# sczhou/CodeFormer

Hardware: AMD Instinct MI355X
Metric: aligned 512x512 faces/sec (whole node) at w=0.5 (higher is better)
Workload: dtype f32; 1 GPU; BASELINE config 2 (IEEE fp32 arithmetic): 16 faces/GPU, w=0.5, adain, seed-0 random-init weights; global_batch=16, parallelism=single GPU, precision=fp32

## Files before the change

### codeformer_amd/archs/codeformer_arch.py

```python
import gc
import os
import threading

import math
import numbers

import numpy as np
import torch
import torch.nn.functional as F
from torch import nn

from .. import ops
from ..ops import EPI_GELU, EPI_RESIDUAL, EPI_SFT, PRO_LEAKY
from ..utils.diagnostics import top2_gap
from ..utils.registry import ARCH_REGISTRY
from .hip_module import PACK_EPOCH, HipModule
from .vqgan_arch import ResBlock, VQAutoEncoder


_GRAPH_LOCK = threading.RLock()
_CAPTURE_STREAMS = {}


def _min_nan(a, b):
# ... 286 lines not shown
    def _encode_hip(self, x, code_only, adain, f43_encoder=None, guard=False, u8=False):
        if u8:
            B = x.shape[0]
        else:
            B, _, Himg, Wimg = x.shape
            if (Himg, Wimg) != (512, 512):
                raise ValueError(f'CodeFormer expects aligned 512x512 faces, got {Himg}x{Wimg}')
            x = x.float().contiguous()
        enc_feat = {}
        enc_taps = {self.fuse_encoder_block[f]: (lambda t: enc_feat.__setitem__(str(t.shape[2]), t))
                    for f in self.connect_list}
        if self.encoder_precision not in ('auto', 'fp32', 'f16x2'):
            raise ValueError(f"encoder_precision must be 'auto', 'fp32' or 'f16x2', got {self.encoder_precision!r}")
        enc_code = ops.SPLIT if self.encoder_precision == 'f16x2' or (self.encoder_precision == 'auto' and self.precision != 'fp32') else ops.WINOGRAD
        if self.winograd_f43_encoder if f43_encoder is None else f43_encoder:
            enc_code = {ops.SPLIT: ops.SPLIT_F43, ops.WINOGRAD: ops.WINOGRAD_F43}[enc_code]
        lq = self.encoder.forward_nhwc(x, enc_taps, bf16=enc_code, img_u8=u8)
        T = lq.shape[1] * lq.shape[2]
        tokens = lq.view(B * T, lq.shape[3])

        if self.gemm_precision not in ('auto', 'fp32', 'f16x2'):
            raise ValueError(f"gemm_precision must be 'auto', 'fp32' or 'f16x2', got {self.gemm_precision!r}")
        gcode = ops.GSPLIT if self.gemm_precision == 'f16x2' else 0
        gcode_ln = ops.GSPLIT if (self.gemm_precision == 'f16x2' or (self.gemm_precision == 'auto' and self.precision != 'fp32' and self.encoder_precision != 'fp32')) else 0
        X = ops.linear(tokens, self._pw_conv('feat_emb', bf16=gcode))
        for layer in self.ft_layers:
            X = layer.forward_tokens(X, self.position_emb, B, code=gcode, code_ln=gcode_ln)
        ln, head = self.idx_pred_layer[0], self.idx_pred_layer[1]
        logits2d = ops.linear(ops.layernorm(X, ln.weight, ln.bias, ln.eps), self._pw_conv(head, bf16=ln_code(self, ln, gcode_ln)))
        res = {'logits': logits2d.view(B, T, -1), 'lq_feat': ops.to_nchw(lq), 'idx': None, 'quant': None, 'enc_feat': enc_feat}
        if guard:
# ... 2 lines not shown
        if code_only:
            return res

        if not guard:
            idx = ops.argmax_rows(logits2d)
            res['idx'] = idx.view(B, T)
        quant = ops.codebook_gather(idx, self.quantize.embedding.weight, B, T,
                                    lq=tokens.view(B, T, -1) if adain else None)
        res['quant'] = quant.view(B, lq.shape[1], lq.shape[2], -1)
        if self.precision not in ('fp32', 'f16x2', 'bf16', 'fp16'):
            raise ValueError(f"precision must be 'fp32', 'f16x2', 'bf16' or 'fp16', got {self.precision!r}")
        return res

    def _generate_hip(self, quant, enc_feat, w, u8=False, out_u8=None):
        B = quant.shape[0]
        bf16 = {'fp32': ops.WINOGRAD_F43, 'f16x2': ops.SPLIT_F43, 'bf16': 1, 'fp16': 2}[self.precision]
        gen_taps = None
        if (torch.is_tensor(w) and w.dim() == 1) or w > 0:
            def fuse(t):
                f = str(t.shape[2])
                enc = enc_feat[f]
                if t.dtype == torch.bfloat16:
                    enc = ops.to_bf16(enc)
                return self.fuse_convs_dict[f].forward_nhwc(enc, t, w, bf16=bf16)
            gen_taps = {self.fuse_generator_block[f]: fuse for f in self.connect_list}
        if u8 and out_u8 is None:
            out_u8 = torch.empty((B, 512, 512, 3), dtype=torch.uint8, device=quant.device)
        return self.generator.forward_nhwc(quant, gen_taps, bf16=bf16, storage_bf16=bool(self.bf16_storage) and bf16 == 1,
                                           img_out=out_u8 if u8 else None)

    def _generate_rows_hip(self, e, w, u8=False, out_u8=None):
# ... 85 lines not shown
            key = (tuple(x.shape), ('per-face', w.fused) if per_face else float(w), bool(code_only), bool(adain), self.precision, bool(self.bf16_storage), self.encoder_precision, self.gemm_precision, bool(self.winograd_f43_encoder), str(x.device), ops.switches(), bool(guard), bool(u8))
            ent = self._graphs.get(key)
            sig = self._param_signature()
            if ent is None or ent['epoch'] != PACK_EPOCH[0] or ent['sig'] != sig:
                static_x = x.clone() if u8 else x.float().contiguous().clone()
                for _ in range(2):
                    self._forward_hip(static_x, w, code_only, adain, guard=guard, u8=u8)
                torch.cuda.synchronize(x.device)
                graph = torch.cuda.CUDAGraph()
                cap = _CAPTURE_STREAMS.get(str(x.device))
                if cap is None:
                    cap = _CAPTURE_STREAMS[str(x.device)] = torch.cuda.Stream(device=x.device)
                with torch.cuda.stream(cap):
                    ops._act_cells(x.device, 4 * max(int(x.shape[0]), 1))
                    ops._counters(x.device, 4096)
                cap.synchronize()
                gc_on = gc.isenabled()
                gc.disable()
                try:
                    with torch.cuda.graph(graph, stream=cap):
                        outs = self._forward_hip(static_x, w, code_only, adain, guard=guard, u8=u8)
                finally:
                    if gc_on:
                        gc.enable()
                ent = {'graph': graph, 'x': static_x, 'outs': outs, 'epoch': PACK_EPOCH[0], 'sig': sig, 'idx': getattr(self, 'last_indices', None),
                       'gap': self.last_min_gap if guard else None, 'w': w if per_face else None}
                self.graph_captures += 1
                self._graphs.pop(key, None)
                while len(self._graphs) >= 4:
                    self._graphs.pop(next(iter(self._graphs)))
# ... 232 lines not shown
```

### codeformer_amd/archs/hip_module.py

```python
import torch
from torch import nn

from .. import ops


PACK_EPOCH = [0]


class HipModule(nn.Module):

    def _packed(self, key, build, *params):
        sig = tuple((p.data_ptr(), ops.tensor_version(p), str(p.device)) for p in params if p is not None)
        cache = self.__dict__.setdefault('_hip_cache', {})
        ent = cache.get(key)
        if ent is None or ent[0] != sig:
            ent = (sig, build())
            cache[key] = ent
            PACK_EPOCH[0] += 1
        return ent[1]

    def _pw_conv(self, name, bf16=False, up2x=False, f16=False, hw=None, c_split=None):
        conv = getattr(self, name) if isinstance(name, str) else name
        code = 2 if f16 else int(bf16)
        if code in (ops.WINOGRAD, ops.WINOGRAD_F43) + ops.SPLIT_CODES or (code in (1, 2) and hw is not None and not up2x):
            cout, cin = conv.weight.shape[:2]
            if hw is None or tuple(conv.weight.shape[2:]) != (3, 3):
                code = 0
            else:
                code = ops.conv_code(code, cin, cout, hw[0], hw[1], up2x=up2x, c_split=c_split)
        key = (name if isinstance(name, str) else id(conv), code, bool(up2x))
        return self._packed(key, lambda: ops.pack_weight(conv.weight, conv.bias, bf16=code, up2x=up2x), conv.weight, conv.bias)

    def _range_code(self, norm, code, n):
        code = int(code)
        if code in (0, 1, ops.WINOGRAD, ops.WINOGRAD_F43):
            return code
        gmax, bmax = self._packed(('gn_range', id(norm)),
                                  lambda: (float(norm.weight.detach().abs().max()), float(norm.bias.detach().abs().max())),
                                  norm.weight, norm.bias)
        return code if ops.gn_range_ok(gmax, bmax, n) else ops.exact_code(code)

    def invalidate_packed_weights(self):
        for m in self.modules():
            if isinstance(m, HipModule):
                m.__dict__.pop('_hip_cache', None)
        PACK_EPOCH[0] += 1

    def forward_nhwc(self, x):
        raise NotImplementedError

# ... 10 lines not shown
```

### codeformer_amd/archs/vqgan_arch.py

```python
import torch
import torch.nn.functional as F
from torch import nn

from .. import ops
from ..ops import EPI_RESIDUAL, PRO_AFFINE, PRO_AFFINE_SWISH
from ..utils.logger import get_root_logger
from ..utils.registry import ARCH_REGISTRY
from .hip_module import HipModule

GN_GROUPS = 32
GN_EPS = 1e-6


def normalize(in_channels):
    return nn.GroupNorm(num_groups=GN_GROUPS, num_channels=in_channels, eps=GN_EPS, affine=True)


def swish(x):
    return x * torch.sigmoid(x)


def _gn_tables(norm, *xs, act_growth=None):
    return ops.groupnorm_tables(list(xs), norm.weight, norm.bias, norm.eps, norm.num_groups, act_growth=act_growth)

# ... 72 lines not shown

    def forward_host(self, x):
        return self.conv(F.pad(x, (0, 1, 0, 1), mode='constant', value=0))


class Upsample(HipModule):

    def __init__(self, in_channels):
        super().__init__()
        self.conv = nn.Conv2d(in_channels, in_channels, kernel_size=3, stride=1, padding=1)

    def forward_nhwc(self, x, bf16=False):
        if int(bf16) == 2:
            bf16 = ops.SPLIT
        c = self.conv.in_channels
        if int(bf16) == ops.WINOGRAD_F43 and x.dtype == torch.float32 and ops.f43_up_ok(c, self.conv.out_channels, 2 * x.shape[1], 2 * x.shape[2]):
            pw = self._packed(('conv', 'f42up'), lambda: ops.pack_weight(self.conv.weight, self.conv.bias, bf16=ops.WF42U), self.conv.weight, self.conv.bias)
            return ops.conv2d(x, pw, upsample=True, emit_stats=True)
        pw = self._pw_conv('conv', bf16, up2x=True, hw=x.shape[1:3])
        return ops.conv2d(x, pw, upsample=True, emit_stats=True, act=ops.act_scale(x) if ops.needs_act_scale(pw) else None)

    def forward_host(self, x):
        return self.conv(F.interpolate(x, scale_factor=2.0, mode='nearest'))


class ResBlock(HipModule):

    def __init__(self, in_channels, out_channels=None):
        super().__init__()
        self.in_channels = in_channels
        self.out_channels = in_channels if out_channels is None else out_channels
# ... 282 lines not shown
```

### codeformer_amd/build.py

```python
import os
import shutil
import subprocess
import sys

PKG = os.path.dirname(os.path.abspath(__file__))
CSRC = os.path.join(PKG, 'csrc')
ROOT = os.path.dirname(PKG)
LIB = os.path.join(PKG, 'libcodeformer_hip.so')
SOURCES = ['cf_igemm.hip', 'cf_winograd.hip', 'cf_split.hip', 'cf_wsplit.hip', 'cf_wf43.hip', 'cf_gemm_split.hip', 'cf_pack.hip', 'cf_norm.hip', 'cf_attention.hip', 'cf_misc.hip', 'cf_paste.hip', 'cf_dcn.hip', 'cf_warp.hip', 'cf_metrics.hip', 'cf_arcface.hip', 'cf_vgg.hip', 'cf_bisenet.hip']


def _hipcc():
    for c in (os.environ.get('HIPCC'), shutil.which('hipcc'), '/opt/rocm/bin/hipcc'):
        if c and os.path.exists(c):
            return c
    raise RuntimeError('hipcc not found (set HIPCC)')


def source_hash():
    import hashlib
    h = hashlib.sha256()
    files = sorted(os.path.join(CSRC, f) for f in os.listdir(CSRC) if f.endswith(('.hip', '.h'))) + \
        [os.path.join(ROOT, 'include', 'codeformer_hip.h')]
    for f in files:
# ... 98 lines not shown
```

### codeformer_amd/csrc/cf_conv_parts.h

```cpp
#pragma once
#include <type_traits>

#include "cf_common.h"

int cf_winograd_launch(const cf_conv_desc* d, hipStream_t stream, int* parts_query, const float* sft_w_img = nullptr);
bool cf_wsplit_covers(const cf_conv_desc* d);
int cf_wsplit_launch(const cf_conv_desc* d, hipStream_t stream, int* parts_query, const float* sft_w_img = nullptr);
int cf_wf43_launch(const cf_conv_desc* d, hipStream_t stream, int* parts_query, const float* sft_w_img = nullptr);
bool cf_wf43_k32(int cout, int cin);
int cf_split_launch(const cf_conv_desc* d, hipStream_t stream, int* parts_query, const float* sft_w_img = nullptr);
int cf_gemm_split_launch(const cf_conv_desc* d, hipStream_t stream, int* parts_query);
int cf_gemm_f32_tile_try(const cf_conv_desc* d, hipStream_t stream);
int cf_gemm_split_geometry(const cf_conv_desc* d, int* tiles, long* bytes_per_part);
int cf_winograd_splitk_geometry(const cf_conv_desc* d, int* tiles, long* bytes_per_part);
int cf_split_splitk_geometry(const cf_conv_desc* d, int* tiles, long* bytes_per_part);

template <class A>
inline void cf_fill_conv_args(A& a, const cf_conv_desc* d, const float* sft_w_img = nullptr) {
  a.in0 = d->in0;
  a.in1 = d->in1;
  a.c0 = d->c0;
  a.c1 = d->c1;
  a.cin = d->c0 + d->c1;
  a.batch = d->batch;
// ... 167 lines not shown
```

### codeformer_amd/csrc/cf_wf43.hip

```cpp
#include <cstdlib>
#include <cstring>
#include <type_traits>

#include "cf_conv_parts.h"




namespace {

constexpr int F4_TH = 16, F4_TW = 16;
constexpr int F4_PW = F4_TW + 2;
constexpr int F4_NPIX = (F4_TH + 2) * F4_PW;
constexpr int F4_SLOTS = F4_NPIX + 4;
constexpr int F4_DUMMY = F4_NPIX;
constexpr int F4_NT = 16;
constexpr int F4_PATCH_FLOATS = F4_SLOTS * CF_BK;
constexpr int F4_PS = F4_NT * CF_BK;
constexpr int F4_V_FLOATS = 36 * F4_PS;
constexpr int F4_M_FLOATS = 36 * 8 * 64;
constexpr int F4_TAB = 256;
constexpr int F4_TAB_32 = 512;
constexpr int F4_LDS_FLOATS = 2 * F4_PATCH_FLOATS + F4_V_FLOATS + 2 * F4_TAB;
static_assert(F4_M_FLOATS <= 2 * F4_PATCH_FLOATS + F4_V_FLOATS, "epilogue staging must fit the patch buffers + V");
// ... 42 lines not shown
  double* stats_out;
  int stats_cpg, nparts;
  int tiles_x, tiles_per_img, ntn;
  int nt_out;
};
static_assert(sizeof(F4Args) == 168, "the kernarg block is 168 bytes (160 before sft_w_img, which found no padding to take): its size feeds the register allocation of every instantiation, so a change is re-checked with tools/kernel_resources.py");

__device__ __forceinline__ int f4_vs(int ty) { return (0x78 >> (2 * ty)) & 3; }

__device__ __forceinline__ unsigned f4_vu(unsigned lq, unsigned p, unsigned t) { return (lq & 1u) + 2u * (((t >> 1) + 4u * (lq >> 1) + p) & 7u); }

template <int PRO, int EPI, int NW, int KS, bool F32, int UPF = 0>
__global__ __launch_bounds__(NW * 64, 4) void wf43_kernel(const F4Args a) {
  constexpr bool UP = UPF == 2;
  constexpr bool GUP = UPF == 1;
  static_assert(UPF == 0 || (F32 && NW == 16 && KS == 32 && PRO == CF_PRO_NONE && EPI == CF_EPI_NONE), "the upsampling forms: fp32 operands on 32-channel slabs, no prologue, no epilogue operand");
  constexpr int NPW = UP ? 13 : 18;
  constexpr int NXI = UP ? 5 : 6;
  constexpr int OS = UP ? 2 : 1;
  static_assert(KS == 16 || (KS == 32 && NW == 16), "32-channel slabs need the LDS of the 16-wave form");
  constexpr int F4_THREADS = NW * 64;
  constexpr int F4_BN = NW * 8;
  constexpr int TWV = KS / 4;
  constexpr int QPP = KS / 4;
  constexpr int GT = F4_THREADS - TWV * 64;
  constexpr int F4_APT = 384 * QPP / GT;
  constexpr int PSTEP = GT / QPP;
  constexpr int SLOTB = KS * 4;
  constexpr int PATCHF = F4_SLOTS * KS;
  constexpr int PSK = F4_NT * KS;
  extern __shared__ __attribute__((aligned(16))) float smem[];
  float* const V = smem + 2 * PATCHF;
  constexpr int VBUF = 36 * PSK;
  constexpr int TABN = KS == 32 ? F4_TAB_32 : F4_TAB;
  float* const tab = V + VBUF;

  const int tid = threadIdx.x;
  const int lane = tid & 63;
  const int wave = __builtin_amdgcn_readfirstlane(tid >> 6);

  const int bid = cf_xcd_tile(blockIdx.x, gridDim.x);
  const int ntile = bid % a.ntn;
  const int mt = bid / a.ntn;
  const int n0 = ntile * F4_BN;
  const int b = mt / a.tiles_per_img;
  const int rt = mt - b * a.tiles_per_img;
  const int blocks = a.tiles_per_img >> 2;
  const int phase = UP ? rt / blocks : 0;
  const int pa = phase >> 1, pb = phase & 1;
  const int blk = UP ? rt - phase * blocks : rt;
  const int tyw = blk / a.tiles_x;
  const int y0 = tyw * F4_TH;
  const int x0 = (blk - tyw * a.tiles_x) * F4_TW;
  const int n = a.cin / KS;

  constexpr bool affine = PRO == CF_PRO_AFFINE || PRO == CF_PRO_AFFINE_SWISH;
  if (affine) {
    for (int i = tid; i < a.cin; i += F4_THREADS) {
      tab[i] = a.pro_scale[(size_t)b * a.cin + i];
      tab[TABN + i] = a.pro_shift[(size_t)b * a.cin + i];
    }
  }
  float act_s, act_is, act_s02;
  cf_act_scales<!affine>(a.act_scale, b, act_s, act_is, act_s02);

  const int py0 = y0 - 1 + pa, px0 = x0 - 1 + pb;
  const int pix_origin = py0 * a.w + px0;
  auto item = [&](unsigned u, int j, unsigned& rel, bool& valid) __attribute__((always_inline)) {
    const unsigned p = u + (unsigned)(PSTEP * j);
    const unsigned hy = (p * 3641u) >> 16;
    const unsigned hx = p - 18u * hy;
    const int iy = py0 + (int)hy, ix = px0 + (int)hx;
    valid = (int)(p < (unsigned)F4_NPIX) & (int)((unsigned)iy < (unsigned)a.h) & (int)((unsigned)ix < (unsigned)a.w);
// ... 346 lines not shown
    asm volatile("" : "+v"(ln));
    lane16 = ln * 32u;
  };
  constexpr std::integral_constant<int, 4> na4{};
  constexpr std::integral_constant<int, 4> na_gather{};
  auto feed = [&](int s) __attribute__((always_inline)) {
    if (s < n) {
      store_patch(s);
    }
  };

  if constexpr (KS == 32) {
    if (wave < TWV) {
      __syncthreads();
      __syncthreads();
      for (int s = 0; s < n; ++s) {
        transform(s, [&]() __attribute__((always_inline)) {
          set_lane32();
          load_B32(s, 0);
        });
        __builtin_amdgcn_sched_barrier(0);
        load_B32(s, 1);
        load_B32(s, 2);
        __builtin_amdgcn_sched_barrier(0);
        __syncthreads();
        mma_stage32(s);
        __builtin_amdgcn_sched_barrier(0);
        __syncthreads();
      }
    } else {
      constexpr std::integral_constant<int, 0> h0{};
      constexpr std::integral_constant<int, F4_APT / 2> h1{};
      constexpr std::integral_constant<int, F4_APT> h2{};
      auto feed2 = [&](int s) __attribute__((always_inline)) {
        if (s < n) {
          load_A_range(s, h1, h2);
          __builtin_amdgcn_sched_barrier(0);
          store_patch_range(s, h0, h1);
          __builtin_amdgcn_sched_barrier(0);
          store_patch_range(s, h1, h2);
        }
      };
      load_A_range(0, h0, h1);
      __syncthreads();
      feed2(0);
      if (n > 1) load_A_range(1, h0, h1);
      __syncthreads();
      for (int s = 0; s < n; ++s) {
        feed2(s + 1);
        __builtin_amdgcn_sched_barrier(0);
        set_lane32();
#pragma unroll
        for (int i = 0; i < 3; ++i) load_B32(s, i);
        __builtin_amdgcn_sched_barrier(0);
        __syncthreads();
        mma_stage32(s);
        __builtin_amdgcn_sched_barrier(0);
        if (s + 2 < n) load_A_range(s + 2, h0, h1);
        __builtin_amdgcn_sched_barrier(0);
        __syncthreads();
      }
    }
  } else if (wave < 4) {
// ... 57 lines not shown
      __builtin_amdgcn_sched_barrier(0);
      __syncthreads();
    }
  }

  float* const Mst = smem;
  const int e_cp = (lane & 31) + 32 * (wave >> 3), e_rh = lane >> 5, e_tp = wave & 7;
  const float acc_s = a.acc_scale * act_is;
  [[maybe_unused]] const float sft_w = EPI == CF_EPI_SFT ? cf_sft_weight(a.sft_w_img, a.sft_w, b) : 0.f;
  const int nn = n0 + 2 * e_cp;
  f4_f32x2 bias2 = {0.f, 0.f};
  if (a.bias) bias2 = *reinterpret_cast<const f4_f32x2*>(a.bias + nn);
  const unsigned e_rowc = (unsigned)(OS * OS * a.w) * (unsigned)a.cout * 4u;
  const unsigned e_px = (unsigned)(OS * a.cout) * 4u;
  const unsigned e_img = (unsigned)(OS * OS) * img_px * (unsigned)a.cout * 4u;
  const __amdgpu_buffer_rsrc_t rs_out = f4_rsrc(a.out + (size_t)(OS * OS) * img0 * a.cout, e_img);
  const __amdgpu_buffer_rsrc_t rs_res = f4_rsrc(EPI == CF_EPI_NONE ? a.out : a.res + img0 * a.cout, e_img);
  const __amdgpu_buffer_rsrc_t rs_sft = f4_rsrc(EPI == CF_EPI_SFT ? a.sft_scale + img0 * a.cout : a.out, e_img);
  const bool rh1 = e_rh != 0;
  const float ca1 = rh1 ? 0.25f : 1.f, ca2 = rh1 ? 4.f : 1.f, cb1 = rh1 ? 0.125f : 0.5f, cb2 = rh1 ? 8.f : 2.f;
  double psum = 0.0, psq = 0.0;
#pragma unroll
  for (int th = 0; th < 2; ++th) {
    unsigned e_zero = 0;
    asm volatile("" : "+v"(e_zero));
    const unsigned voff0 = (unsigned)(2 * e_rh) * e_rowc + (unsigned)(2 * e_cp) * 4u + e_zero;
    const unsigned soff0 = (unsigned)(y0 + 4 * (e_tp >> 1)) * e_rowc + (unsigned)(x0 + 4 * (2 * th + (e_tp & 1))) * e_px + (unsigned)n0 * 4u +
                           (UP ? (unsigned)(pa * 2 * a.w + pb) * (unsigned)a.cout * 4u : 0u);
    f4_f32x2 r0[2][4], r1[2][4];
#pragma unroll
    for (int aa = 0; aa < 2; ++aa)
// ... 68 lines not shown
#pragma unroll
      for (int aa = 0; aa < 2; ++aa) {
        const f4_f32x2 s = ta[aa] + tb[aa], d = ta[aa] - tb[aa];
        o[aa][0] += s;
        o[aa][1] += d * 2.f;
        o[aa][2] += s * 4.f;
        o[aa][3] += d * 8.f + t0[aa];
      }
    }
    double dsum = 0.0, dsq = 0.0, dsum1 = 0.0, dsq1 = 0.0;
#pragma unroll
    for (int aa = 0; aa < 2; ++aa) {
      f4_f32x2 rs = {0.f, 0.f}, rq = {0.f, 0.f};
#pragma unroll
      for (int c = 0; c < 4; ++c) {
        f4_f32x2 v = o[aa][c] * acc_s + bias2;
        if (EPI == CF_EPI_RESIDUAL) v += r0[aa][c];
        else if (EPI == CF_EPI_SFT) v = r0[aa][c] + sft_w * (r0[aa][c] * r1[aa][c] + v);
        o[aa][c] = v;
        rs += v;
        rq += v * v;
      }
      dsum += (double)rs[0];
      dsq += (double)rq[0];
      dsum1 += (double)rs[1];
      dsq1 += (double)rq[1];
    }
    if (a.nt_out) {
#pragma unroll
      for (int aa = 0; aa < 2; ++aa)
#pragma unroll
// ... 66 lines not shown
  CF_REQUIRE(!sub || (d->hin % F4_TH == 0 && d->win % F4_TW == 0 && d->hout == 2 * d->hin && d->wout == 2 * d->win),
             "cf_conv2d(winograd 2, upsample 2): needs an input of %dx%d multiples (got %dx%d)", F4_TH, F4_TW, d->hin, d->win);
  if (!f32)
    if (const int e = cf_require_acc_scale(d, "cf_conv2d(winograd 2)")) return e;
  CF_REQUIRE(!f32 || !d->act_scale, "cf_conv2d(winograd 2): fp32 operands take no activation range scale");
  CF_REQUIRE(d->hout % F4_TH == 0 && d->wout % F4_TW == 0, "cf_conv2d(winograd 2): needs an output of %dx%d multiples (got %dx%d)", F4_TH,
             F4_TW, d->hout, d->wout);
  CF_REQUIRE(d->cout % 64 == 0 && d->cout_pad == d->cout, "cf_conv2d(winograd 2): needs cout == cout_pad, a multiple of 64 (got %d / %d)",
             d->cout, d->cout_pad);
  CF_REQUIRE((long)d->hout * d->wout <= (1L << 21), "cf_conv2d(winograd 2): at most 2^21 pixels per image (got %dx%d)", d->hout, d->wout);
  CF_REQUIRE((long)d->hout * d->wout * (d->c0 > d->cout ? d->c0 : d->cout) * 4 < (1L << 31) && (long)d->hout * d->wout * d->c1 * 4 < (1L << 31),
             "cf_conv2d(winograd 2): an image of a tensor must stay below 2^31 bytes (%dx%d, %d / %d / %d channels)", d->hout, d->wout, d->c0, d->c1, d->cout);
  const int tab_max = cf_wf43_k32(d->cout, d->c0 + d->c1) ? F4_TAB_32 : F4_TAB;
  CF_REQUIRE(d->c0 + d->c1 <= tab_max, "cf_conv2d(winograd 2): at most %d input channels in this form (got %d)", tab_max, d->c0 + d->c1);
  CF_REQUIRE(cf_epi_is_quad_triple(d), "cf_conv2d(winograd 2): epilogues are none / residual / SFT");
  CF_REQUIRE(cf_dense_zero_pad(d) && d->split_k < 1, "cf_conv2d(winograd 2): reads / writes dense tensors with zero padding, no split_k");
  CF_REQUIRE(d->stats_cpg == 0 || (d->stats_cpg <= 64 && (d->stats_cpg & (d->stats_cpg - 1)) == 0 && d->stats_cpg >= 2),
             "cf_conv2d(winograd 2): stats_cpg %d (a power of two, 2..64)", d->stats_cpg);
  F4Args a;
  cf_fill_conv_args(a, d, sft_w_img);
  a.nchunks = a.cin / CF_BK;
  a.h = d->hout;
  a.w = d->wout;
  a.acc_scale = f32 ? 1.f : d->acc_scale;
  a.act_scale = d->act_scale;
  a.stats_cpg = d->stats_cpg > 0 ? d->stats_cpg : 2;
  a.tiles_x = d->wout / F4_TW;
  a.tiles_per_img = a.tiles_x * (d->hout / F4_TH);
  a.nparts = a.tiles_per_img;
  const bool wide = d->cout % 128 == 0;
  const bool k32 = cf_wf43_k32(d->cout, d->c0 + d->c1);
// ... 7 lines not shown
  }
  if (parts_query) {
    *parts_query = a.nparts;
    return CF_OK;
  }
  const size_t lds = (k32 ? F4_LDS_FLOATS_32 : wide ? F4_LDS_FLOATS_16 : F4_LDS_FLOATS) * sizeof(float);
  const dim3 grid(a.tiles_per_img * d->batch * a.ntn), block(wide ? 1024 : 512);
  if (d->upsample) {
    CF_LDS_ATTR((wf43_kernel<CF_PRO_NONE, CF_EPI_NONE, 16, 32, true, 1>), F4_LDS_FLOATS_32 * sizeof(float));
    CF_LDS_ATTR((wf43_kernel<CF_PRO_NONE, CF_EPI_NONE, 16, 32, true, 2>), F4_LDS_FLOATS_32 * sizeof(float));
    if (sub) hipLaunchKernelGGL((wf43_kernel<CF_PRO_NONE, CF_EPI_NONE, 16, 32, true, 2>), grid, block, lds, stream, a);
    else hipLaunchKernelGGL((wf43_kernel<CF_PRO_NONE, CF_EPI_NONE, 16, 32, true, 1>), grid, block, lds, stream, a);
    CF_CHECK_LAUNCH("cf_conv2d(winograd F(4,3) / F(4,2) fp32, upsampling forms)");
    return CF_OK;
  }
  auto launch = [&](auto pro, auto epi, auto op) {
    constexpr int P = decltype(pro)::value, E = decltype(epi)::value;
    constexpr bool O = decltype(op)::value;
    CF_LDS_ATTR((wf43_kernel<P, E, 8, 16, O>), F4_LDS_FLOATS * sizeof(float));
    CF_LDS_ATTR((wf43_kernel<P, E, 16, 16, O>), F4_LDS_FLOATS_16 * sizeof(float));
    CF_LDS_ATTR((wf43_kernel<P, E, 16, 32, O>), F4_LDS_FLOATS_32 * sizeof(float));
    if (k32) hipLaunchKernelGGL((wf43_kernel<P, E, 16, 32, O>), grid, block, lds, stream, a);
    else if (wide) hipLaunchKernelGGL((wf43_kernel<P, E, 16, 16, O>), grid, block, lds, stream, a);
    else hipLaunchKernelGGL((wf43_kernel<P, E, 8, 16, O>), grid, block, lds, stream, a);
  };
  cf_with_prologue(d->prologue, [&](auto pro) {
    cf_with_epilogue(d->epilogue, [&](auto epi) {
      if (f32) launch(pro, epi, std::true_type{});
      else launch(pro, epi, std::false_type{});
    });
  });
// ... 4 lines not shown
```

### codeformer_amd/ops.py

```python
import ctypes
import math
import os
import weakref

import torch

from . import lib as L
from .lib import (EPI_AXPY, EPI_AXPY2, EPI_GELU, EPI_LEAKY, EPI_NONE, EPI_PRELU, EPI_RES_PRELU, EPI_RESIDUAL, EPI_SFT, PRO_AFFINE, PRO_AFFINE_SWISH,
                  PAD_EDGE, PAD_REFLECT, PAD_ZERO, PRO_LEAKY, PRO_NONE)

GN_GROUPS = 32
GN_EPS = 1e-6

PROFILE = None


def _f32(t):
    if t.dtype != torch.float32:
        raise TypeError(f'expected float32, got {t.dtype}')
    return t


def _act_dtype(t, what='activation'):
    if t.dtype not in (torch.float32, torch.bfloat16):
# ... 55 lines not shown

    def __init__(self, part, parts, cpg, stamp=None):
        self.part, self.parts, self.cpg, self.stamp = part, parts, cpg, stamp


def select_rows(x, sel):
    y = x.index_select(0, sel)
    st = live_stats(x)
    if st is not None:
        y._cf_stats = GNStats(st.part.view(x.shape[0], -1).index_select(0, sel).reshape(-1), st.parts, st.cpg, tensor_stamp(y))
    return y


class PackedWeight:

    __slots__ = ('w', 'bias', 'cout', 'cin', 'taps', 'cout_pad', 'cin_pad', 'bf16', 'up2x', 'wino', 'scale', 's2', 'conv1')

    def __init__(self, w, bias, cout, cin, taps, cout_pad, cin_pad, bf16=False, up2x=False, wino=False, scale=1.0, s2=False, conv1=False):
        self.w, self.bias, self.cout, self.cin, self.taps = w, bias, cout, cin, taps
        self.cout_pad, self.cin_pad, self.bf16, self.up2x, self.wino = cout_pad, cin_pad, bf16, up2x, wino
        self.s2 = s2
        self.conv1 = conv1
        self.scale = scale


def _cout_pad(cout):
    if cout <= 32:
        return 32
    if cout <= 64:
        return 64
    return (cout + 127) // 128 * 128


WINOGRAD = 3
SPLIT = 4
WSPLIT = 6
GSPLIT = 7
WF16 = 8
WBF16 = 9
SPLIT_F43 = 10
WF43 = 11
WINOGRAD_F43 = 12
WF43F = 13
WF42U = 14
OPERAND_F16X2 = 3
SPLIT_CODES = (SPLIT, SPLIT_F43)


def split_ok(cin, cout, hin, win, c_split=None):
    return cin % 32 == 0 and cout % 64 == 0 and hin % 16 == 0 and win % 16 == 0 and (c_split is None or c_split % 32 == 0)


def split_s2_ok(cin, cout, hin, win):
    return cin % 16 == 0 and cout % 64 == 0 and hin % 16 == 0 and win % 32 == 0


def split_1x1_ok(cin, cout, h, w, c_split=None):
    return cin % 32 == 0 and cout % 64 == 0 and h % 8 == 0 and w % 16 == 0 and h * w > TOKEN_IMAGE_MAX and (c_split is None or c_split % 32 == 0)

# ... 1 lines not shown
def winograd_ok(cin, cout, hout, wout):
    return cin % 16 == 0 and cout % 64 == 0 and hout % 8 == 0 and wout % 16 == 0


F43_WIDE_MIN_PIXELS = 128 * 128
F43_WIDE_MIN_PIXELS_FP32 = 64 * 64


def f43_ok(cin, cout, hout, wout, fp32=False):
    if cout != 64 and (cout % 128 or hout * wout < (F43_WIDE_MIN_PIXELS_FP32 if fp32 else F43_WIDE_MIN_PIXELS)):
        return False
    cin_max = 512 if (cout % 128 == 0 and cin % 32 == 0) else 256
    return cin % 16 == 0 and cin <= cin_max and cout % 64 == 0 and hout % 16 == 0 and wout % 16 == 0




def f43_up_ok(cin, cout, hout, wout):
    return cin % 32 == 0 and cin <= 256 and cout % 128 == 0 and hout % 32 == 0 and wout % 32 == 0 and \
        hout * wout >= F43_WIDE_MIN_PIXELS_FP32


SPLIT_MIN_PIXELS = 32 * 32
TOKEN_IMAGE_MAX = 1024


def wsingle_ok(cin, cout, h, w):
    return winograd_ok(cin, cout, h, w) and cout % 128 == 0 and h * w >= SPLIT_MIN_PIXELS


def c_split_ok(c_split, slab):
    return c_split is None or c_split % slab == 0


def conv_code(code, cin, cout, h, w, up2x=False, c_split=None, plain=True):
    code = int(code)
    f43_slab = 32 if (cout % 128 == 0 and cin % 32 == 0) else 16
    if code == WINOGRAD_F43:
        if plain and not up2x and c_split_ok(c_split, f43_slab) and f43_ok(cin, cout, h, w, fp32=True):
            return WF43F
        code = WINOGRAD
    if code == SPLIT_F43:
        if plain and not up2x and c_split_ok(c_split, f43_slab) and f43_ok(cin, cout, h, w):
            return WF43
        code = SPLIT
    if code == SPLIT:
        if plain and not up2x and winograd_ok(cin, cout, h, w):
            return WSPLIT
        if plain and split_ok(cin, cout, h, w, c_split) and (up2x or h * w >= SPLIT_MIN_PIXELS):
            return SPLIT
        code = WINOGRAD
    if code == WINOGRAD:
# ... 147 lines not shown
    if up2x or w.dim() != 4 or tuple(w.shape[2:]) != (3, 3) or w.shape[1] % cin_mult or w.shape[0] % cout_mult:
        raise ValueError(f'{what} packing needs a 3x3 weight with cin % {cin_mult} == 0 and cout % {cout_mult} == 0 (and has no up2x form)')


def _packed(name, n, w, *args, dtype=torch.float32):
    packed = torch.empty(n, dtype=dtype, device=w.device)
    L.check(getattr(L.load(), name)(L.ptr(w), *args, L.ptr(packed, dtype=None), L.stream_ptr()), name)
    return packed


_WINO = {WINOGRAD: ('winograd', 'cf_pack_conv_weight_winograd', 16, None, False, True),
         WSPLIT: ('winograd f16x2', 'cf_pack_conv_weight_winograd_f16x2', 16, _f23_max, OPERAND_F16X2, True),
         WF16: ('winograd f16x2', 'cf_pack_conv_weight_winograd_f16x2', 16, _f23_max, 2, True),
         WBF16: ('winograd f16x2', 'cf_pack_conv_weight_winograd_bf16', 16, _f23_max, 1, True),
         WF43F: ('winograd F(4,3)', 'cf_pack_conv_weight_winograd43', 36, None, False, 2),
         WF42U: ('winograd F(4,2) sub-pixel', 'cf_pack_conv_weight_winograd42_up', 100, None, False, 2),
         WF43: ('winograd F(4,3) f16x2', 'cf_pack_conv_weight_winograd43_f16x2', 36, _f43_max, OPERAND_F16X2, 2)}


def _pack_winograd(w, b, code, up2x, stride2):
    what, fn, npos, domain_max, operand, wino = _WINO[code]
    up = code == WF42U
    _require_3x3(w, 32 if up else 16, 128 if up else 64, what, up2x)
    cout, cin = w.shape[:2]
    scale = () if domain_max is None else (pack_scale(domain_max(w)),)
    return PackedWeight(_packed(fn, npos * cin * cout, w, cout, cin, cout, cin, *scale), b, cout, cin, 9, cout, cin, bf16=operand, up2x=up, wino=wino, scale=(*scale, 1.0)[0])


def _pack_split(w, b, code, up2x, stride2):
    cout, cin, conv1 = w.shape[0], w.shape[1], w.dim() == 2 or tuple(w.shape[2:]) == (1, 1)
    if conv1 and (up2x or cin % 32 or cout % 64):
        raise ValueError('f16x2 1x1 packing needs cin % 32 == 0 and cout % 64 == 0')
    if not conv1:
        _require_3x3(w, 16 if stride2 else 32, 64, 'f16x2', False)
    form = 3 if conv1 else 2 if stride2 else int(bool(up2x))
    scale = pack_scale(float(w.abs().max()) * (4.0 if up2x else 1.0))
    packed = _packed('cf_pack_conv_weight_f16x2', (9, 16, 16, 1)[form] * cin * cout, w, cout, cin, form, cout, cin, scale)
    return PackedWeight(packed, b, cout, cin, 1 if conv1 else 9, cout, cin, bf16=OPERAND_F16X2, up2x=bool(up2x), scale=scale, s2=bool(stride2) and not conv1, conv1=conv1)


def _pack_gemm_split(w, b, code, up2x, stride2):
# ... 73 lines not shown
        if int(pw.bf16) == OPERAND_F16X2 and not pw.conv1 and batch * ho * wo * pw.cout_pad <= GEMM_IN_WG_MAX_OUTPUTS and cin <= 1024:
            return SPLITK_IN_WORKGROUP
        tiles = batch * (ho * wo // 64) * (pw.cout_pad // 64)
    else:
        return 0
    cap = 256 if pw.wino else 128
    v = cin // 128
    for ns in (8, 4, 2):
        if ns <= SPLITK_MAX and v % ns == 0 and tiles * ns <= cap:
            return ns
    return 1


def _counters(device, n):
    return _scratch(_COUNTERS, device, n, 4096)


def _roofline_kind(pw, io, stride, upsample, c0, in_nchw, out_nchw, out_pixels, split_k):
    kind = ('conv3x3_s2' if stride == 2 else ('conv_up2x' if upsample else ('conv3x3_wino' if pw.wino else 'conv3x3'))) if pw.taps == 9 else 'gemm1x1'
    if pw.taps == 9 and stride == 1 and ((in_nchw and c0 <= 4) or (out_nchw and pw.cout <= 4)):
        kind = 'conv3x3_io'
    if pw.bf16:
        kind += ('', '_bf16', '_f16', '_f16x2')[int(pw.bf16)]
    if io == torch.bfloat16 and not pw.bf16:
        kind += '_bf16io'
    if pw.conv1:
        kind = 'conv1x1_stream_f16x2'
    if pw.wino == 2:
        return 'conv3x3_wino43_f16x2' if pw.bf16 else 'conv3x3_wino43'
    return kind + ('_8w' if pw.wino and pw.bf16 and pw.cout % 128 == 0 and out_pixels >= 1024 and not split_k else '')
# ... 92 lines not shown
        in0=None if img_in is not None else L.ptr(x, not in_nchw, dtype=io), in1=L.ptr(x2, True, dtype=io), c0=c0, c1=c1, batch=B, hin=H, win=W, hout=Ho, wout=Wo, cout=pw.cout,
        cout_pad=pw.cout_pad, taps=pw.taps, stride=stride, upsample=2 if f42_up else int(bool(upsample)), in_nchw=int(bool(in_nchw)),
        out_nchw=int(bool(out_nchw)), prologue=prologue, epilogue=epilogue, pro_scale=L.ptr(scale),
        pro_shift=L.ptr(shift), weight=L.ptr(pw.w, dtype=None), bias=L.ptr(pw.bias), res=L.ptr(res, True, dtype=io),
        sft_scale=L.ptr(sft_scale, True, dtype=io), sft_w=float(sft_w), out=None if img_out is not None else L.ptr(out, not out_nchw, dtype=odt), bf16_mfma=int(pw.bf16),
        ld_in0=ld0, ld_in1=ld1, ld_out=ldo, pad_mode=int(pad_mode), pad_lo=int(pad_lo), winograd=int(pw.wino),
        acc_scale=1.0 / pw.scale, io_bf16=int(io == torch.bfloat16))
    if x_alt is not None:
        if tuple(x_alt.shape) != tuple(x.shape) or x_alt.dtype != torch.float32 or int(pw.bf16) != OPERAND_F16X2 or pw.taps != 1 or pw.conv1 or x2 is not None:
            raise ValueError('x_alt: a second float32 token matrix of the same shape, for a split-half token GEMM (bf16=GSPLIT weight)')
        d.in0_alt, d.alt_cout0 = L.ptr(x_alt), int(alt_from)
    if act is not None and needs_act_scale(pw):
        if tuple(act.shape) != (B, 2) or prologue not in (PRO_NONE, PRO_LEAKY):
            raise ValueError('act: expected a (B, 2) table and a none / leaky prologue')
        d.act_scale = L.ptr(act)
    if split_k is None:
        dense = not in_nchw and not out_nchw and ld0 == c0 and (c1 == 0 or ld1 == c1) and ldo in (0, pw.cout)
        split_k = splitk_for(pw, Ho, Wo, c0 + c1, B) if (stride == 1 and dense) else 0
    if split_k:
        d.split_k = int(split_k)
        if split_k > 1:
            nbytes, tiles = lib.cf_conv2d_workspace_bytes(ctypes.byref(d)), lib.cf_conv2d_tiles(ctypes.byref(d))
            if nbytes < 0 or tiles <= 0:
                raise RuntimeError(f'cf_conv2d_workspace_bytes failed: {L.last_error()}')
            ws = torch.empty(nbytes // 4, dtype=torch.float32, device=dev)
            d.workspace, d.counters = L.ptr(ws), L.ptr(_counters(dev, tiles), dtype=torch.int32)
    stats = None
    if emit_stats and not out_nchw and pw.cout % GN_GROUPS == 0 and pw.cout // GN_GROUPS >= 2:
        d.stats_cpg = pw.cout // GN_GROUPS
        parts = lib.cf_conv2d_stats_parts(ctypes.byref(d))
        if parts <= 0:
# ... 907 lines not shown
```

Before: 352.9 faces/s.

## Add K-split Winograd F(4,3) fp32 path with separate partial-sum epilogue kernel

Adds a K-parts form of the fp32 Winograd F(4,3) conv for mid-sized layers (256-512 input channels, small spatial sizes). Each workgroup handles one 128-channel slice of the input channels and writes its partial result into a workspace plane. A new reduction kernel then sums the planes and applies bias, residual/SFT and GroupNorm stats. The aim is more workgroups on small-resolution layers that would otherwise underfill the GPU. The cost is extra workspace traffic and one more kernel launch per conv.

```diff
diff --git a/codeformer_amd/archs/codeformer_arch.py b/codeformer_amd/archs/codeformer_arch.py
--- a/codeformer_amd/archs/codeformer_arch.py
+++ b/codeformer_amd/archs/codeformer_arch.py
@@ -324,7 +324,7 @@
             raise ValueError(f"encoder_precision must be 'auto', 'fp32' or 'f16x2', got {self.encoder_precision!r}")
         enc_code = ops.SPLIT if self.encoder_precision == 'f16x2' or (self.encoder_precision == 'auto' and self.precision != 'fp32') else ops.WINOGRAD
         if self.winograd_f43_encoder if f43_encoder is None else f43_encoder:
-            enc_code = {ops.SPLIT: ops.SPLIT_F43, ops.WINOGRAD: ops.WINOGRAD_F43}[enc_code]
+            enc_code = {ops.SPLIT: ops.SPLIT_F43, ops.WINOGRAD: ops.WINOGRAD_F43K}[enc_code]
         lq = self.encoder.forward_nhwc(x, enc_taps, bf16=enc_code, img_u8=u8)
         T = lq.shape[1] * lq.shape[2]
         tokens = lq.view(B * T, lq.shape[3])
@@ -357,7 +357,7 @@
 
     def _generate_hip(self, quant, enc_feat, w, u8=False, out_u8=None):
         B = quant.shape[0]
-        bf16 = {'fp32': ops.WINOGRAD_F43, 'f16x2': ops.SPLIT_F43, 'bf16': 1, 'fp16': 2}[self.precision]
+        bf16 = {'fp32': ops.WINOGRAD_F43K,'f16x2': ops.SPLIT_F43, 'bf16': 1, 'fp16': 2}[self.precision]
         gen_taps = None
         if (torch.is_tensor(w) and w.dim() == 1) or w > 0:
             def fuse(t):
@@ -473,6 +473,8 @@
                 with torch.cuda.stream(cap):
                     ops._act_cells(x.device, 4 * max(int(x.shape[0]), 1))
                     ops._counters(x.device, 4096)
+                    if self.precision == 'fp32':
+                        ops._kpart_ws(x.device, max(int(x.shape[0]), 1) << 20)
                 cap.synchronize()
                 gc_on = gc.isenabled()
                 gc.disable()
diff --git a/codeformer_amd/archs/hip_module.py b/codeformer_amd/archs/hip_module.py
--- a/codeformer_amd/archs/hip_module.py
+++ b/codeformer_amd/archs/hip_module.py
@@ -22,7 +22,7 @@
     def _pw_conv(self, name, bf16=False, up2x=False, f16=False, hw=None, c_split=None):
         conv = getattr(self, name) if isinstance(name, str) else name
         code = 2 if f16 else int(bf16)
-        if code in (ops.WINOGRAD, ops.WINOGRAD_F43) + ops.SPLIT_CODES or (code in (1, 2) and hw is not None and not up2x):
+        if code in (ops.WINOGRAD,) + ops.F43_FP32_CODES + ops.SPLIT_CODES or (code in (1, 2) and hw is not None and not up2x):
             cout, cin = conv.weight.shape[:2]
             if hw is None or tuple(conv.weight.shape[2:]) != (3, 3):
                 code = 0
@@ -33,7 +33,7 @@
 
     def _range_code(self, norm, code, n):
         code = int(code)
-        if code in (0, 1, ops.WINOGRAD, ops.WINOGRAD_F43):
+        if code in (0, 1, ops.WINOGRAD) + ops.F43_FP32_CODES:
             return code
         gmax, bmax = self._packed(('gn_range', id(norm)),
                                   lambda: (float(norm.weight.detach().abs().max()), float(norm.bias.detach().abs().max())),
diff --git a/codeformer_amd/archs/vqgan_arch.py b/codeformer_amd/archs/vqgan_arch.py
--- a/codeformer_amd/archs/vqgan_arch.py
+++ b/codeformer_amd/archs/vqgan_arch.py
@@ -110,7 +110,7 @@
         if int(bf16) == 2:
             bf16 = ops.SPLIT
         c = self.conv.in_channels
-        if int(bf16) == ops.WINOGRAD_F43 and x.dtype == torch.float32 and ops.f43_up_ok(c, self.conv.out_channels, 2 * x.shape[1], 2 * x.shape[2]):
+        if int(bf16) in ops.F43_FP32_CODES and x.dtype == torch.float32 and ops.f43_up_ok(c, self.conv.out_channels, 2 * x.shape[1], 2 * x.shape[2]):
             pw = self._packed(('conv', 'f42up'), lambda: ops.pack_weight(self.conv.weight, self.conv.bias, bf16=ops.WF42U), self.conv.weight, self.conv.bias)
             return ops.conv2d(x, pw, upsample=True, emit_stats=True)
         pw = self._pw_conv('conv', bf16, up2x=True, hw=x.shape[1:3])
diff --git a/codeformer_amd/build.py b/codeformer_amd/build.py
--- a/codeformer_amd/build.py
+++ b/codeformer_amd/build.py
@@ -7,7 +7,7 @@
 CSRC = os.path.join(PKG, 'csrc')
 ROOT = os.path.dirname(PKG)
 LIB = os.path.join(PKG, 'libcodeformer_hip.so')
-SOURCES = ['cf_igemm.hip', 'cf_winograd.hip', 'cf_split.hip', 'cf_wsplit.hip', 'cf_wf43.hip', 'cf_gemm_split.hip', 'cf_pack.hip', 'cf_norm.hip', 'cf_attention.hip', 'cf_misc.hip', 'cf_paste.hip', 'cf_dcn.hip', 'cf_warp.hip', 'cf_metrics.hip', 'cf_arcface.hip', 'cf_vgg.hip', 'cf_bisenet.hip']
+SOURCES = ['cf_igemm.hip', 'cf_winograd.hip', 'cf_split.hip', 'cf_wsplit.hip', 'cf_wf43.hip', 'cf_ksum.hip', 'cf_gemm_split.hip', 'cf_pack.hip', 'cf_norm.hip', 'cf_attention.hip', 'cf_misc.hip', 'cf_paste.hip', 'cf_dcn.hip', 'cf_warp.hip', 'cf_metrics.hip', 'cf_arcface.hip', 'cf_vgg.hip', 'cf_bisenet.hip']
 
 
 def _hipcc():
diff --git a/codeformer_amd/csrc/cf_conv_parts.h b/codeformer_amd/csrc/cf_conv_parts.h
--- a/codeformer_amd/csrc/cf_conv_parts.h
+++ b/codeformer_amd/csrc/cf_conv_parts.h
@@ -7,6 +7,7 @@
 bool cf_wsplit_covers(const cf_conv_desc* d);
 int cf_wsplit_launch(const cf_conv_desc* d, hipStream_t stream, int* parts_query, const float* sft_w_img = nullptr);
 int cf_wf43_launch(const cf_conv_desc* d, hipStream_t stream, int* parts_query, const float* sft_w_img = nullptr);
+int cf_ksum_launch(const cf_conv_desc* d, hipStream_t stream, const float* sft_w_img);
 bool cf_wf43_k32(int cout, int cin);
 int cf_split_launch(const cf_conv_desc* d, hipStream_t stream, int* parts_query, const float* sft_w_img = nullptr);
 int cf_gemm_split_launch(const cf_conv_desc* d, hipStream_t stream, int* parts_query);
diff --git a/codeformer_amd/csrc/cf_ksum.hip b/codeformer_amd/csrc/cf_ksum.hip
--- /dev/null
+++ b/codeformer_amd/csrc/cf_ksum.hip
@@ -0,0 +1,135 @@
+#include "cf_conv_parts.h"
+
+namespace {
+
+struct KSumArgs {
+  const float* ws;
+  const float* bias;
+  const float* res;
+  const float* sft_scale;
+  const float* sft_w_img;
+  float* out;
+  double* stats_out;
+  float sft_w, acc_scale;
+  int parts, batch, h, w, cout;
+  int epilogue, stats_cpg;
+  int tiles_x, tiles_per_img, nblk;
+  int nt_out;
+};
+
+template <int CB>
+__global__ __launch_bounds__(256) void ksum_kernel(const KSumArgs a) {
+  constexpr int Q4 = CB / 4;
+  constexpr int PSTEP = 256 / Q4;
+  constexpr int NIT = 256 / PSTEP;
+  __shared__ double sred[4][Q4][4];
+  const int tid = threadIdx.x, lane = tid & 63, wave = tid >> 6;
+  const int bid = blockIdx.x;
+  const int nb = bid % a.nblk;
+  const int mt = bid / a.nblk;
+  const int b = mt / a.tiles_per_img;
+  const int rt = mt - b * a.tiles_per_img;
+  const int ty = rt / a.tiles_x;
+  const int y0 = ty * 16, x0 = (rt - ty * a.tiles_x) * 16;
+  const int quad = tid % Q4, p0 = tid / Q4;
+  const int n = nb * CB + quad * 4;
+  const size_t plane = (size_t)a.batch * a.h * a.w * a.cout;
+  f32x4 bias4 = {0.f, 0.f, 0.f, 0.f};
+  if (a.bias) bias4 = *reinterpret_cast<const f32x4*>(a.bias + n);
+  const float sft_w = a.epilogue == CF_EPI_SFT ? cf_sft_weight(a.sft_w_img, a.sft_w, b) : 0.f;
+  const bool nt = a.nt_out != 0;
+  double s01 = 0.0, s23 = 0.0, q01 = 0.0, q23 = 0.0;
+#pragma unroll 4
+  for (int k = 0; k < NIT; ++k) {
+    const int p = p0 + k * PSTEP;
+    const size_t off = (((size_t)b * a.h + (y0 + (p >> 4))) * a.w + (x0 + (p & 15))) * a.cout + n;
+    f32x4 r0 = {0.f, 0.f, 0.f, 0.f}, r1 = {0.f, 0.f, 0.f, 0.f};
+    if (a.epilogue == CF_EPI_RESIDUAL || a.epilogue == CF_EPI_SFT) r0 = *reinterpret_cast<const f32x4*>(a.res + off);
+    if (a.epilogue == CF_EPI_SFT) r1 = *reinterpret_cast<const f32x4*>(a.sft_scale + off);
+    f32x4 v = {0.f, 0.f, 0.f, 0.f};
+    for (int c = 0; c < a.parts; ++c) v += *reinterpret_cast<const f32x4*>(a.ws + (size_t)c * plane + off);
+    v = cf_epi_bias<true>(v, a.acc_scale, bias4);
+    v = cf_epi_apply(v, a.epilogue, r0, r1, sft_w);
+    cf_store16(a.out + off, v, nt);
+    const double d0 = v[0], d1 = v[1], d2 = v[2], d3 = v[3];
+    s01 += d0 + d1;
+    s23 += d2 + d3;
+    q01 += d0 * d0 + d1 * d1;
+    q23 += d2 * d2 + d3 * d3;
+  }
+  if (!a.stats_out) return;
+  const int cpg = a.stats_cpg;
+  double d0 = s01, q0 = q01, d1 = s23, q1 = q23;
+  if (cpg != 2) {
+    d0 += d1;
+    q0 += q1;
+  }
+  for (int o = Q4; o < 64; o <<= 1) {
+    d0 += __shfl_xor(d0, o, 64);
+    q0 += __shfl_xor(q0, o, 64);
+    d1 += __shfl_xor(d1, o, 64);
+    q1 += __shfl_xor(q1, o, 64);
+  }
+  for (int o = 1; o * 4 < cpg; o <<= 1) {
+    d0 += __shfl_xor(d0, o, 64);
+    q0 += __shfl_xor(q0, o, 64);
+  }
+  if (lane < Q4) {
+    sred[wave][lane][0] = d0;
+    sred[wave][lane][1] = q0;
+    sred[wave][lane][2] = d1;
+    sred[wave][lane][3] = q1;
+  }
+  __syncthreads();
+  if (tid < Q4 && (n % cpg) == 0) {
+    double t[4] = {0.0, 0.0, 0.0, 0.0};
+#pragma unroll
+    for (int wv = 0; wv < 4; ++wv)
+#pragma unroll
+      for (int e = 0; e < 4; ++e) t[e] += sred[wv][tid][e];
+    double* op = cf_gn_partial_ptr(a.stats_out, b, a.cout, cpg, n, a.tiles_per_img, rt);
+    op[0] = t[0];
+    op[1] = t[1];
+    if (cpg == 2) {
+      op[(size_t)a.tiles_per_img * 2] = t[2];
+      op[(size_t)a.tiles_per_img * 2 + 1] = t[3];
+    }
+  }
+}
+
+}
+
+int cf_ksum_launch(const cf_conv_desc* d, hipStream_t stream, const float* sft_w_img) {
+  CF_REQUIRE(d->workspace && d->split_k >= 2 && d->hout % 16 == 0 && d->wout % 16 == 0 && d->cout % 64 == 0 && cf_epi_is_quad_triple(d),
+             "cf_conv2d(K-part sum): needs a workspace of split_k >= 2 planes, whole 16x16 patches, cout %% 64 == 0, epilogue none / residual / SFT");
+  CF_REQUIRE(d->epilogue == CF_EPI_NONE || d->res, "cf_conv2d(K-part sum): the residual / SFT epilogue needs res");
+  CF_REQUIRE(d->epilogue != CF_EPI_SFT || d->sft_scale, "cf_conv2d(K-part sum): the SFT epilogue needs sft_scale");
+  KSumArgs a;
+  a.ws = d->workspace;
+  a.bias = d->bias;
+  a.res = d->res;
+  a.sft_scale = d->sft_scale;
+  a.sft_w_img = sft_w_img;
+  a.out = d->out;
+  a.stats_out = d->stats_out;
+  a.sft_w = d->sft_w;
+  a.acc_scale = 1.f;
+  a.parts = d->split_k;
+  a.batch = d->batch;
+  a.h = d->hout;
+  a.w = d->wout;
+  a.cout = d->cout;
+  a.epilogue = d->epilogue;
+  a.stats_cpg = d->stats_cpg > 0 ? d->stats_cpg : 2;
+  a.tiles_x = d->wout / 16;
+  a.tiles_per_img = a.tiles_x * (d->hout / 16);
+  a.nt_out = cf_nt_store((long)d->batch * d->hout * d->wout * d->cout * 4);
+  const bool wide = d->stats_out && a.stats_cpg == 64;
+  const int cb = wide ? 64 : 32;
+  a.nblk = d->cout / cb;
+  const dim3 grid(d->batch * a.tiles_per_img * a.nblk), block(256);
+  if (wide) hipLaunchKernelGGL(ksum_kernel<64>, grid, block, 0, stream, a);
+  else hipLaunchKernelGGL(ksum_kernel<32>, grid, block, 0, stream, a);
+  CF_CHECK_LAUNCH("cf_conv2d(K-part sum)");
+  return CF_OK;
+}
diff --git a/codeformer_amd/csrc/cf_wf43.hip b/codeformer_amd/csrc/cf_wf43.hip
--- a/codeformer_amd/csrc/cf_wf43.hip
+++ b/codeformer_amd/csrc/cf_wf43.hip
@@ -80,7 +80,8 @@
 __global__ __launch_bounds__(NW * 64, 4) void wf43_kernel(const F4Args a) {
   constexpr bool UP = UPF == 2;
   constexpr bool GUP = UPF == 1;
-  static_assert(UPF == 0 || (F32 && NW == 16 && KS == 32 && PRO == CF_PRO_NONE && EPI == CF_EPI_NONE), "the upsampling forms: fp32 operands on 32-channel slabs, no prologue, no epilogue operand");
+  constexpr bool KP = UPF == 3;
+  static_assert(UPF == 0 || (F32 && NW == 16 && KS == 32 && (PRO == CF_PRO_NONE || KP) && EPI == CF_EPI_NONE), "the upsampling forms: fp32 operands on 32-channel slabs, no prologue, no epilogue operand; the K-part form: any prologue");
   constexpr int NPW = UP ? 13 : 18;
   constexpr int NXI = UP ? 5 : 6;
   constexpr int OS = UP ? 2 : 1;
@@ -107,7 +108,10 @@
 
   const int bid = cf_xcd_tile(blockIdx.x, gridDim.x);
   const int ntile = bid % a.ntn;
-  const int mt = bid / a.ntn;
+  const int kparts = KP ? a.cin / (4 * KS) : 1;
+  const int mtp = bid / a.ntn;
+  const int part = KP ? mtp % kparts : 0;
+  const int mt = KP ? mtp / kparts : mtp;
   const int n0 = ntile * F4_BN;
   const int b = mt / a.tiles_per_img;
   const int rt = mt - b * a.tiles_per_img;
@@ -118,11 +122,12 @@
   const int tyw = blk / a.tiles_x;
   const int y0 = tyw * F4_TH;
   const int x0 = (blk - tyw * a.tiles_x) * F4_TW;
-  const int n = a.cin / KS;
+  const int s0 = KP ? 4 * part : 0;
+  const int n = KP ? s0 + 4 : a.cin / KS;
 
   constexpr bool affine = PRO == CF_PRO_AFFINE || PRO == CF_PRO_AFFINE_SWISH;
   if (affine) {
-    for (int i = tid; i < a.cin; i += F4_THREADS) {
+    for (int i = tid + s0 * KS; i < (KP ? n * KS : a.cin); i += F4_THREADS) {
       tab[i] = a.pro_scale[(size_t)b * a.cin + i];
       tab[TABN + i] = a.pro_shift[(size_t)b * a.cin + i];
     }
@@ -499,7 +504,7 @@
     if (wave < TWV) {
       __syncthreads();
       __syncthreads();
-      for (int s = 0; s < n; ++s) {
+      for (int s = s0; s < n; ++s) {
         transform(s, [&]() __attribute__((always_inline)) {
           set_lane32();
           load_B32(s, 0);
@@ -526,12 +531,12 @@
           store_patch_range(s, h1, h2);
         }
       };
-      load_A_range(0, h0, h1);
+      load_A_range(s0, h0, h1);
       __syncthreads();
-      feed2(0);
-      if (n > 1) load_A_range(1, h0, h1);
+      feed2(s0);
+      if (n > s0 + 1) load_A_range(s0 + 1, h0, h1);
       __syncthreads();
-      for (int s = 0; s < n; ++s) {
+      for (int s = s0; s < n; ++s) {
         feed2(s + 1);
         __builtin_amdgcn_sched_barrier(0);
         set_lane32();
@@ -619,7 +624,7 @@
   const unsigned e_rowc = (unsigned)(OS * OS * a.w) * (unsigned)a.cout * 4u;
   const unsigned e_px = (unsigned)(OS * a.cout) * 4u;
   const unsigned e_img = (unsigned)(OS * OS) * img_px * (unsigned)a.cout * 4u;
-  const __amdgpu_buffer_rsrc_t rs_out = f4_rsrc(a.out + (size_t)(OS * OS) * img0 * a.cout, e_img);
+  const __amdgpu_buffer_rsrc_t rs_out = f4_rsrc(a.out + ((size_t)(OS * OS) * img0 + (KP ? (size_t)part * a.batch * img_px : (size_t)0)) * a.cout, e_img);
   const __amdgpu_buffer_rsrc_t rs_res = f4_rsrc(EPI == CF_EPI_NONE ? a.out : a.res + img0 * a.cout, e_img);
   const __amdgpu_buffer_rsrc_t rs_sft = f4_rsrc(EPI == CF_EPI_SFT ? a.sft_scale + img0 * a.cout : a.out, e_img);
   const bool rh1 = e_rh != 0;
@@ -718,7 +723,7 @@
       f4_f32x2 rs = {0.f, 0.f}, rq = {0.f, 0.f};
 #pragma unroll
       for (int c = 0; c < 4; ++c) {
-        f4_f32x2 v = o[aa][c] * acc_s + bias2;
+        f4_f32x2 v = KP ? o[aa][c] : o[aa][c] * acc_s + bias2;
         if (EPI == CF_EPI_RESIDUAL) v += r0[aa][c];
         else if (EPI == CF_EPI_SFT) v = r0[aa][c] + sft_w * (r0[aa][c] * r1[aa][c] + v);
         o[aa][c] = v;
@@ -815,7 +820,12 @@
   const int tab_max = cf_wf43_k32(d->cout, d->c0 + d->c1) ? F4_TAB_32 : F4_TAB;
   CF_REQUIRE(d->c0 + d->c1 <= tab_max, "cf_conv2d(winograd 2): at most %d input channels in this form (got %d)", tab_max, d->c0 + d->c1);
   CF_REQUIRE(cf_epi_is_quad_triple(d), "cf_conv2d(winograd 2): epilogues are none / residual / SFT");
-  CF_REQUIRE(cf_dense_zero_pad(d) && d->split_k < 1, "cf_conv2d(winograd 2): reads / writes dense tensors with zero padding, no split_k");
+  const bool kp = d->split_k >= 2;
+  CF_REQUIRE(cf_dense_zero_pad(d) && (d->split_k < 1 || kp), "cf_conv2d(winograd 2): reads / writes dense tensors with zero padding, no split_k but the K-part form's cin / 128");
+  CF_REQUIRE(!kp || (f32 && !d->upsample && !d->io_bf16 && d->cout % 128 == 0 && (d->c0 + d->c1) % 128 == 0 && d->c0 + d->c1 <= 512 && d->c0 % 128 == 0 &&
+                     d->split_k == (d->c0 + d->c1) / 128 && (parts_query || d->workspace)),
+             "cf_conv2d(winograd 2, K parts): fp32 operands, cout %% 128 == 0, cin %% 128 == 0 and <= 512, a concat boundary on a multiple of 128, split_k == cin / 128 "
+             "(got %d for cin %d) and a workspace of split_k x batch x hout x wout x cout floats", d->split_k, d->c0 + d->c1);
   CF_REQUIRE(d->stats_cpg == 0 || (d->stats_cpg <= 64 && (d->stats_cpg & (d->stats_cpg - 1)) == 0 && d->stats_cpg >= 2),
              "cf_conv2d(winograd 2): stats_cpg %d (a power of two, 2..64)", d->stats_cpg);
   F4Args a;
@@ -853,7 +863,24 @@
     CF_CHECK_LAUNCH("cf_conv2d(winograd F(4,3) / F(4,2) fp32, upsampling forms)");
     return CF_OK;
   }
-  auto launch = [&](auto pro, auto epi, auto op) {
+  if (kp) {
+    CF_REQUIRE(k32, "cf_conv2d(winograd 2, K parts): runs on 32-channel slabs only (CF_F43_WIDE=k16 is set)");
+    F4Args p = a;
+    p.out = d->workspace;
+    p.epilogue = CF_EPI_NONE;
+    p.bias = p.res = p.sft_scale = nullptr;
+    p.stats_out = nullptr;
+    p.nt_out = 0;
+    const dim3 pgrid(grid.x * d->split_k);
+    cf_with_prologue(d->prologue, [&](auto pro) {
+      constexpr int P = decltype(pro)::value;
+      CF_LDS_ATTR((wf43_kernel<P, CF_EPI_NONE, 16, 32, true, 3>), F4_LDS_FLOATS_32 * sizeof(float));
+      hipLaunchKernelGGL((wf43_kernel<P, CF_EPI_NONE, 16, 32, true, 3>), pgrid, block, lds, stream, p);
+    });
+    CF_CHECK_LAUNCH("cf_conv2d(winograd F(4,3) fp32, K parts)");
+    return cf_ksum_launch(d, stream, sft_w_img);
+  }
+  auto launch =[&](auto pro, auto epi, auto op) {
     constexpr int P = decltype(pro)::value, E = decltype(epi)::value;
     constexpr bool O = decltype(op)::value;
     CF_LDS_ATTR((wf43_kernel<P, E, 8, 16, O>), F4_LDS_FLOATS * sizeof(float));
diff --git a/codeformer_amd/ops.py b/codeformer_amd/ops.py
--- a/codeformer_amd/ops.py
+++ b/codeformer_amd/ops.py
@@ -93,10 +93,11 @@
 
 class PackedWeight:
 
-    __slots__ = ('w', 'bias', 'cout', 'cin', 'taps', 'cout_pad', 'cin_pad', 'bf16', 'up2x', 'wino', 'scale', 's2', 'conv1')
-
-    def __init__(self, w, bias, cout, cin, taps, cout_pad, cin_pad, bf16=False, up2x=False, wino=False, scale=1.0, s2=False, conv1=False):
+    __slots__ = ('w', 'bias', 'cout', 'cin', 'taps', 'cout_pad', 'cin_pad', 'bf16', 'up2x', 'wino', 'scale', 's2', 'conv1', 'kparts')
+
+    def __init__(self, w, bias, cout, cin, taps, cout_pad, cin_pad, bf16=False, up2x=False, wino=False, scale=1.0, s2=False, conv1=False, kparts=0):
         self.w, self.bias, self.cout, self.cin, self.taps = w, bias, cout, cin, taps
+        self.kparts = kparts
         self.cout_pad, self.cin_pad, self.bf16, self.up2x, self.wino = cout_pad, cin_pad, bf16, up2x, wino
         self.s2 = s2
         self.conv1 = conv1
@@ -122,6 +123,9 @@
 WINOGRAD_F43 = 12
 WF43F = 13
 WF42U = 14
+WINOGRAD_F43K = 15
+WF43K = 16
+F43_FP32_CODES = (WINOGRAD_F43, WINOGRAD_F43K)
 OPERAND_F16X2 = 3
 SPLIT_CODES = (SPLIT, SPLIT_F43)
 
@@ -153,6 +157,18 @@
     return cin % 16 == 0 and cin <= cin_max and cout % 64 == 0 and hout % 16 == 0 and wout % 16 == 0
 
 
+F43K_MIN_WORKGROUPS = 16
+
+
+def f43k_ok(cin, cout, hout, wout, c_split=None):
+    return f43k_covers(cin, cout, hout, wout, c_split) and (hout // 16) * (wout // 16) * (cin // 128) * (cout // 128) >= F43K_MIN_WORKGROUPS
+
+
+def f43k_covers(cin, cout, hout, wout, c_split=None):
+    return cout % 128 == 0 and cin % 128 == 0 and 256 <= cin <= 512 and hout % 16 == 0 and wout % 16 == 0 and 256 <= hout * wout < F43_WIDE_MIN_PIXELS_FP32 and \
+        (c_split is None or c_split % 128 == 0)
+
+
 
 
 def f43_up_ok(cin, cout, hout, wout):
@@ -175,6 +191,10 @@
 def conv_code(code, cin, cout, h, w, up2x=False, c_split=None, plain=True):
     code = int(code)
     f43_slab = 32 if (cout % 128 == 0 and cin % 32 == 0) else 16
+    if code == WINOGRAD_F43K:
+        if plain and not up2x and f43k_ok(cin, cout, h, w, c_split):
+            return WF43K
+        code = WINOGRAD_F43
     if code == WINOGRAD_F43:
         if plain and not up2x and c_split_ok(c_split, f43_slab) and f43_ok(cin, cout, h, w, fp32=True):
             return WF43F
@@ -352,6 +372,7 @@
          WF16: ('winograd f16x2', 'cf_pack_conv_weight_winograd_f16x2', 16, _f23_max, 2, True),
          WBF16: ('winograd f16x2', 'cf_pack_conv_weight_winograd_bf16', 16, _f23_max, 1, True),
          WF43F: ('winograd F(4,3)', 'cf_pack_conv_weight_winograd43', 36, None, False, 2),
+         WF43K: ('winograd F(4,3) K parts', 'cf_pack_conv_weight_winograd43', 36, None, False, 2),
          WF42U: ('winograd F(4,2) sub-pixel', 'cf_pack_conv_weight_winograd42_up', 100, None, False, 2),
          WF43: ('winograd F(4,3) f16x2', 'cf_pack_conv_weight_winograd43_f16x2', 36, _f43_max, OPERAND_F16X2, 2)}
 
@@ -359,10 +380,14 @@
 def _pack_winograd(w, b, code, up2x, stride2):
     what, fn, npos, domain_max, operand, wino = _WINO[code]
     up = code == WF42U
-    _require_3x3(w, 32 if up else 16, 128 if up else 64, what, up2x)
+    kp = code == WF43K
+    _require_3x3(w, 128 if kp else 32 if up else 16, 128 if (up or kp) else 64, what, up2x)
     cout, cin = w.shape[:2]
+    if kp and not 256 <= cin <= 512:
+        raise ValueError(f'{what} packing needs 2 .. 4 parts of 128 input channels (got cin {cin})')
     scale = () if domain_max is None else (pack_scale(domain_max(w)),)
-    return PackedWeight(_packed(fn, npos * cin * cout, w, cout, cin, cout, cin, *scale), b, cout, cin, 9, cout, cin, bf16=operand, up2x=up, wino=wino, scale=(*scale, 1.0)[0])
+    return PackedWeight(_packed(fn, npos * cin * cout, w, cout, cin, cout, cin, *scale), b, cout, cin, 9, cout, cin, bf16=operand, up2x=up, wino=wino, scale=(*scale, 1.0)[0],
+                        kparts=cin // 128 if kp else 0)
 
 
 def _pack_split(w, b, code, up2x, stride2):
@@ -466,6 +491,13 @@
 
 def _counters(device, n):
     return _scratch(_COUNTERS, device, n, 4096)
+
+
+_KPART_WS = {}
+
+
+def _kpart_ws(device, n):
+    return _scratch(_KPART_WS, device, n, 1 << 22)
 
 
 def _roofline_kind(pw, io, stride, upsample, c0, in_nchw, out_nchw, out_pixels, split_k):
@@ -588,7 +620,14 @@
         if tuple(act.shape) != (B, 2) or prologue not in (PRO_NONE, PRO_LEAKY):
             raise ValueError('act: expected a (B, 2) table and a none / leaky prologue')
         d.act_scale = L.ptr(act)
-    if split_k is None:
+    if pw.kparts:
+        dense = not in_nchw and not out_nchw and ld0 == c0 and (c1 == 0 or ld1 == c1) and ldo in (0, pw.cout)
+        if split_k or upsample or stride != 1 or not dense or io != torch.float32 or not f43k_covers(c0 + c1, pw.cout, Ho, Wo, c0 if c1 else None):
+            raise ValueError('a weight packed with bf16=WF43K serves dense fp32 3x3 stride-1 launches of the shapes f43k_covers names (conv_code decides: pack with its answer)')
+        d.split_k = pw.kparts
+        d.workspace = L.ptr(_kpart_ws(dev, pw.kparts * B * Ho * Wo * pw.cout), dtype=torch.int32)
+        split_k = 0
+    elif split_k is None:
         dense = not in_nchw and not out_nchw and ld0 == c0 and (c1 == 0 or ld1 == c1) and ldo in (0, pw.cout)
         split_k = splitk_for(pw, Ho, Wo, c0 + c1, B) if (stride == 1 and dense) else 0
     if split_k:
```

Result: faster. 360.0 faces/s, median of 6 (+2.0%).
